# Dao-AILab/flash-attention

Hardware: AMD Instinct MI355X
Metric: attention_fwd_tflops (higher is better)
Workload: dtype bf16; 1 GPU; BASELINE config 3: B=4 H=32 S=4096 D=128 bf16 causal, forward (flash_attn_func path, fa_fwd via C ABI); batch=4, heads=32, seqlen=4096, head_dim=128, causal=True, parallelism=replicas x1

## Files before the change

### flash-attention_amd/csrc/fa_bwd_dkdv_w64.hip

```cpp
#include <cstdlib>
#include <type_traits>

#include "fa_device.h"
#include "fa_kernel_params.h"
#include "fa_launch.h"
#include "fa_fwd_w64_regs.h"
#define FA_W64_CLOB FA_W64_ACC_CLOBBERS_256
#include "fa_w64_asm.h"

#define FA_DKDV64_AHJ 6
#define FA_DKDV64_AHT 3

#ifndef FA_DKDV64_PART
#define FA_DKDV64_PART 0
#endif

namespace fa {
namespace {

template <typename E> FA_DEVINL void kv_mfma_c0(f32x16& d, u32x4 a, u32x4 b) {
  if constexpr (std::is_same<E, __bf16>::value)
    asm volatile("v_mfma_f32_32x32x16_bf16 %0, %1, %2, 0" : "=&v"(d) : "v"(a), "v"(b) : FA_W64_CLOB);
  else
    asm volatile("v_mfma_f32_32x32x16_f16 %0, %1, %2, 0" : "=&v"(d) : "v"(a), "v"(b) : FA_W64_CLOB);
// ... 521 lines not shown
        if constexpr (g == 1) stream_dma_q(c.z);
        if constexpr (g == 3) stream_dma_d(c.z);
        if constexpr (DS && g >= 5 && g <= 11 && (g & 1) == 1) ds_store(ICw<(g - 5) / 2>{});
      });
    } else {
      stream_dma_q(c.z); stream_dma_d(c.z);
      if constexpr (DS) static_for<4>(ds_store);
#pragma unroll
      for (int kb = 0; kb < KB; ++kb)
#pragma unroll
        for (int t = 0; t < 2; ++t) { pc[kb][t] = pn[kb][t]; dc[kb][t] = dn[kb][t]; }
    }
    using Y = ICw<1>; using N = ICw<0>;
    const bool had_prev = c.slot_b != c.slot_a;
    if (__builtin_expect(c.act || had_prev, 1)) {
      if (__builtin_expect(!had_prev, 0)) {
#pragma unroll
        for (int kb = 0; kb < KB; ++kb)
#pragma unroll
          for (int t = 0; t < 2; ++t)
#pragma unroll
            for (int i = 0; i < 4; ++i) {
              unsigned z0, z1;
              asm volatile("v_mov_b32 %0, 0\n\tv_mov_b32 %1, 0" : "=v"(z0), "=v"(z1));
              pc[kb][t][i] = z0; dc[kb][t][i] = z1;
            }
      }
      if (__builtin_expect(c.act && c.msk, 0)) phase_b(Y{}, Y{}, Y{}, c.slot_b, c.q0, pc, dc, pn, dn, c.slot_a);
      else phase_b(Y{}, Y{}, N{}, c.slot_b, c.q0, pc, dc, pn, dn, c.slot_a);
    }
    lds_dma_wait_all();
    stream_store_aux(c.slot2);
    __builtin_amdgcn_sched_barrier(0);
    const int hq_n = (ALIBI || DS) ? (c_left == 1 ? c_h + 1 : c_h) : 0;
    preload_a((st + 1) & 3, hq_n);
    __builtin_amdgcn_sched_barrier(0);
    advance(c, st);
    __builtin_amdgcn_sched_barrier(0);
    __syncthreads();
  };
#pragma unroll 1
  for (int st = 0; st <= n_steps; ++st) step(st);

  char FA_LDS* stage = lds + wave * 32 * (ROW_BYTES + 16);
  mfma_drain_acc();
  static_for<KB>([&](auto kbc) __attribute__((always_inline)) {
    constexpr int kb = decltype(kbc)::value;
    const int kb0 = wk0 + 32 * kb;
    if (kb0 < sk) {
      E* dktile = (E*)p.dk + dk_boff + (k_row0 + kb0) * p.dk_rs + (int64_t)hk * p.dk_hs;
      E* dvtile = (E*)p.dv + dv_boff + (k_row0 + kb0) * p.dv_rs + (int64_t)hk * p.dv_hs;
      f32x16 tt[DB];
      static_for<DB>([&](auto dbc) __attribute__((always_inline)) { acc_read_tuple<16 * (2 * DB + kb * DB + decltype(dbc)::value)>(tt[decltype(dbc)::value]); });
      store_tile_via_lds<E, D>(stage, tt, CAP ? 4.f * p.scale : p.scale, dktile, p.dk_rs, sk - kb0, lane);
      static_for<DB>([&](auto dbc) __attribute__((always_inline)) { acc_read_tuple<16 * (kb * DB + decltype(dbc)::value)>(tt[decltype(dbc)::value]); });
      store_tile_via_lds<E, D>(stage, tt, 1.f, dvtile, p.dv_rs, sk - kb0, lane);
    }
  });
}

#if FA_DKDV64_PART != 2
template <typename E, int D, int FEAT>
__global__ void __launch_bounds__(256, 1) fa_bwd_dkdv_w64_kernel(const BwdK p) {
  dkdv_w64_body<E, D, FEAT, false>(p, blockIdx.x);
}
#endif

#if FA_DKDV64_PART != 1
template <typename E, int D>
static __device__ __forceinline__ void dq_ds_w64_body(const BwdK p, const int cbid) {
  using T = ElemTraits<E>;
  using V8 = typename T::v8;
  constexpr int NW = 4, QB = 2, BM = NW * 64, BN = 64, CPR = D / 8;
  constexpr int ROW_BYTES = D * 2, TILE_K = BN * ROW_BYTES, DB = D / 32;
  constexpr int DS_WAVE = QB * 2 * 2048;
  constexpr int SLOT = TILE_K + NW * DS_WAVE, RING = 3;
  constexpr int RPD = 1024 / ROW_BYTES, DPW = TILE_K / 1024 / NW;
  static_assert(DPW == 4 || DPW == 2, "K pieces per wave");

  extern __shared__ __attribute__((aligned(16))) char smem[];
  char FA_LDS* lds = (char FA_LDS*)smem;
  const int tid = threadIdx.x, lane = tid & 63;
  const int wave = __builtin_amdgcn_readfirstlane(tid >> 6);
  const int hi = lane >> 5;

  const int xcd = cbid & 7, slot_i = cbid >> 3;
  const int per_unit = p.hk_ratio * p.nmb;
  const int jr = slot_i / per_unit, within = slot_i - jr * per_unit;
  const int hg = within / p.nmb, mbr = within - hg * p.nmb;
  const int j = p.c5_cj0 + jr;
  int unit;
  if (p.k_unit_hpx > 0) { const int bb = j / p.k_unit_hpx; unit = bb * (8 * p.k_unit_hpx) + xcd * p.k_unit_hpx + (j - bb * p.k_unit_hpx); }
  else unit = xcd + 8 * j;
  if (unit >= p.k_units) return;
  const int b = unit / p.h_k, hk = unit - b * p.h_k;
  const int h = hk * p.hk_ratio + hg;
  const int m_block = (p.wr >= 0) ? (p.nmb - 1 - mbr) : mbr;
  const int sq = p.sq, sk = p.sk, shift = sk - sq;
  const int m0 = m_block * BM;
  if (m0 >= sq) return;
  const int blk_last = min(m0 + BM, sq) - 1;
  const int kmax = (p.wr >= 0) ? min(sk - 1, blk_last + shift + p.wr) : sk - 1;
  const int n_max = kmax >= 0 ? kmax / BN + 1 : 0;
  const int w_row0 = m0 + wave * 64;

  const E* __restrict__ kp = (const E*)p.k + (int64_t)b * p.k_bs + (int64_t)hk * p.k_hs;
  auto make_srd = [&](const void* base, unsigned long long bytes) __attribute__((always_inline)) {
    const unsigned long long a = (unsigned long long)base;
    u32x4 sd = {(unsigned)__builtin_amdgcn_readfirstlane((unsigned)a), (unsigned)__builtin_amdgcn_readfirstlane((unsigned)(a >> 32)) & 0xffffu,
// ... 89 lines not shown
    if (__builtin_expect(n < n_all, 1)) {
      static_for<4>([&](auto ksc) __attribute__((always_inline)) {
        constexpr int ks = decltype(ksc)::value, kb = ks >> 1, t = ks & 1;
        u32x4 bf[QB];
#pragma unroll
        for (int qb = 0; qb < QB; ++qb) {
          const int a = DOFF + ds_lane + qb * 4096 + kb * 2048 + t * 512;
          bf[qb] = rd_tr(a, a + 256);
        }
        static_for<DB>([&](auto dbc) __attribute__((always_inline)) {
          constexpr int db = decltype(dbc)::value;
          constexpr int kbase = KOFF + kb * 32 * ROW_BYTES + 16 * t * ROW_BYTES;
          const u32x4 af = rd_tr(kbase + (tr_base[0] ^ (db << 6)), kbase + (tr_base[1] ^ (db << 6)));
          kv_mfma_tile<E, db>(af, bf[0]);
          kv_mfma_tile<E, DB + db>(af, bf[1]);
        });
      });
    } else {
      static_for<4>([&](auto ksc) __attribute__((always_inline)) {
        constexpr int ks = decltype(ksc)::value, kb = ks >> 1, t = ks & 1;
        const bool a0 = ds_tile_active(w_row0, n * BN + 32 * kb, sq, sk, shift, p.wl, p.wr), a1 = ds_tile_active(w_row0 + 32, n * BN + 32 * kb, sq, sk, shift, p.wl, p.wr);
        if (a0 || a1) {
          u32x4 bf[QB];
#pragma unroll
          for (int qb = 0; qb < QB; ++qb) {
            const int a = DOFF + ds_lane + qb * 4096 + kb * 2048 + t * 512;
            bf[qb] = rd_tr(a, a + 256);
          }
          static_for<DB>([&](auto dbc) __attribute__((always_inline)) {
            constexpr int db = decltype(dbc)::value;
            constexpr int kbase = KOFF + kb * 32 * ROW_BYTES + 16 * t * ROW_BYTES;
            const u32x4 af = rd_tr(kbase + (tr_base[0] ^ (db << 6)), kbase + (tr_base[1] ^ (db << 6)));
            if (a0) kv_mfma_tile<E, db>(af, bf[0]);
            if (a1) kv_mfma_tile<E, DB + db>(af, bf[1]);
          });
        }
      });
    }
  };
  for (int n = 0; n < n_max; n += RING) {
    tile(ICw<0>{}, n);
    if (n + 1 < n_max) tile(ICw<1>{}, n + 1);
    if (n + 2 < n_max) tile(ICw<2>{}, n + 2);
  }
  __syncthreads();
  mfma_drain_acc();
  E* dqtile = (E*)p.dq + (int64_t)b * p.dq_bs + (int64_t)w_row0 * p.dq_rs + (int64_t)h * p.dq_hs;
  static_for<QB>([&](auto qbc) __attribute__((always_inline)) {
    constexpr int qb = decltype(qbc)::value;
    const int row0 = w_row0 + 32 * qb;
    f32x16 tt[DB];
    static_for<DB>([&](auto dbc) __attribute__((always_inline)) { acc_read_tuple<16 * (qb * DB + decltype(dbc)::value)>(tt[decltype(dbc)::value]); });
    if (row0 < sq)
      store_tile_via_lds<E, D>(lds + (wave * 64 + qb * 32) * (ROW_BYTES + 16), tt, p.scale, dqtile + (int64_t)(32 * qb) * p.dq_rs, p.dq_rs, sq - row0, lane);
  });
}

template <typename E, int D>
__global__ void __launch_bounds__(256, 1) fa_bwd_c5_kernel(const BwdK p) {
  const int bid = blockIdx.x;
  if (bid < p.c5_np) dkdv_w64_body<E, D, 0, true>(p, bid + p.c5_pbid0);
  else dq_ds_w64_body<E, D>(p, bid - p.c5_np);
}

template <typename E, int D>
static int launch_c5_t(const BwdK& p, hipStream_t stream) {
  constexpr int dkdv = 4 * 2 * 32 * D * 2 + 256 * D * 2 + 4 * 2 * 32 * 4 + (D == 128 ? 4 * (D / 16 - 1) * 1024 : 0);
  constexpr int dq = 3 * (64 * D * 2 + 4 * 8192), stage = 256 * (D * 2 + 16);
  constexpr int smem = dkdv > dq ? (dkdv > stage ? dkdv : stage) : (dq > stage ? dq : stage);
  static_assert(smem <= 160 * 1024, "LDS");
  auto kern = fa_bwd_c5_kernel<E, D>;
  static std::atomic<unsigned long long> attr_mask{0};
  if (ensure_dyn_lds(attr_mask, (const void*)kern, 160 * 1024, true) != 0) return -1;
  const long long total = (long long)p.c5_np + p.c5_nc;
  if (total <= 0) return 0;
  hipLaunchKernelGGL(kern, dim3((unsigned)total), dim3(256), smem, stream, p);
  return hipGetLastError() == hipSuccess ? 0 : -1;
}

int launch_bwd_c5(const BwdK& p, int dtype_bf16, int d, hipStream_t stream) {
  if (p.rng != nullptr || p.alibi != nullptr || p.softcap > 0.f || p.d_chunks > 0 || p.cu_q || p.cu_k || p.seqused_q || p.seqused_k || p.k_list) return -2;
  if (p.wl >= 0 || p.sk < p.sq || (d != 128 && d != 64) || (p.c5_np > 0 && !p.ds_ws) || (p.c5_nc > 0 && !p.ds_rd)) return -2;
  const uint64_t span = ((uint64_t)(p.sq > 0 ? p.sq : 1) + 64) * (uint64_t)(p.q_rs > p.do_rs ? p.q_rs : p.do_rs) * 2u;
  const uint64_t kspan = ((uint64_t)p.sk + 128) * (uint64_t)p.k_rs * 2u;
  if (span >= (1ull << 32) || kspan >= (1ull << 32)) return -2;
  if (d == 128) return dtype_bf16 ? launch_c5_t<__bf16, 128>(p, stream) : launch_c5_t<_Float16, 128>(p, stream);
  return dtype_bf16 ? launch_c5_t<__bf16, 64>(p, stream) : launch_c5_t<_Float16, 64>(p, stream);
}
#endif

#if FA_DKDV64_PART != 2
template <typename E, int D, int FEAT>
static int launch_dkdv_w64_f(const BwdK& p, hipStream_t stream) {
  constexpr bool ALIBI = FEAT == FEAT_ALIBI;
  constexpr int base = 4 * 2 * 32 * D * 2 + 256 * D * 2 + 4 * 2 * 32 * 4 + (D == 128 ? 4 * (D / 16 - 1) * 1024 : 0);
  const int smem = base + (ALIBI ? (4 * (p.hk_ratio + 1) + 15) / 16 * 16 : 0);
  if (smem > 160 * 1024) return -2;
  auto kern = fa_bwd_dkdv_w64_kernel<E, D, FEAT>;
  static std::atomic<unsigned long long> attr_mask{0};
  if (ensure_dyn_lds(attr_mask, (const void*)kern, 160 * 1024, true) != 0) return -1;
  const long long total = p.k_list ? (long long)p.k_bound * p.h_k : units_grid(p.k_units, p.k_unit_size);
  if (total <= 0) return 0;
  hipLaunchKernelGGL(kern, dim3((unsigned)total), dim3(256), smem, stream, p);
  return hipGetLastError() == hipSuccess ? 0 : -1;
}
template <typename E, int D>
static int launch_dkdv_w64_t(const BwdK& p, hipStream_t stream) {
// ... 19 lines not shown
```

### flash-attention_amd/csrc/fa_bwd_w64.hip

```cpp
#include <cstdio>
#include <cstdlib>
#include <type_traits>

#include "fa_device.h"
#include "fa_kernel_params.h"
#include "fa_launch.h"
#include "fa_fwd_w64_regs.h"
#define FA_W64_CLOB FA_W64_ACC_CLOBBERS_256
#include "fa_w64_asm.h"

#define FA_BW64_AH 2

namespace fa {
namespace {

constexpr int BW_Q_BASE = 128;
constexpr int BW_DO_BASE = 192;
constexpr float kLog2eW = 1.4426950408889634f;

template <typename E, int BASE> FA_DEVINL void mfma_v_first(f32x16& d, u32x4 a, const f32x16& c) {
  if constexpr (std::is_same<E, __bf16>::value)
    asm volatile("v_mfma_f32_32x32x16_bf16 %0, %1, a[%c3:%c4], %2" : "=&v"(d) : "v"(a), "v"(c), "i"(BASE), "i"(BASE + 3) : FA_W64_CLOB);
  else
    asm volatile("v_mfma_f32_32x32x16_f16 %0, %1, a[%c3:%c4], %2" : "=&v"(d) : "v"(a), "v"(c), "i"(BASE), "i"(BASE + 3) : FA_W64_CLOB);
// ... 560 lines not shown
  auto generic_iter = [&](int u) __attribute__((always_inline)) {
    iter_head(u);
    generic_step(ICw<0>{}, 2 * u - 1, sA, dpA, sB, dpB, fA, fB);
    generic_step(ICw<1>{}, 2 * u, sB, dpB, sA, dpA, fB, fA);
    iter_tail();
  };
  if (n_tiles > 0) {
    int u = 0;
    const int head_end = min(max(uf_lo, 0), n_tiles + 1);
    for (; u < head_end; ++u) generic_iter(u);
    const unsigned wave_dst = (unsigned)(wave * DPW * 1024);
    auto fast_iter = [&](auto maskc, int uu) __attribute__((always_inline)) {
      const int nslot = slot_k == RING - 1 ? 0 : slot_k + 1;
      const unsigned toff_k = (unsigned)(n_min + uu + 1) * (unsigned)(BN * 2) * (unsigned)p.k_rs;
      const unsigned toff_v = (unsigned)(n_min + uu + 1) * (unsigned)(BN * 2) * (unsigned)p.v_rs;
      u32x4 fring[AHK + 1];
      fast_step(ICw<0>{}, maskc, 2 * uu - 1, sA, dpA, sB, dpB, fA, fB, k_srd, koff_l, toff_k,
                __builtin_amdgcn_readfirstlane((unsigned)(nslot * TILE_BYTES) + wave_dst), fring);
      fast_step(ICw<1>{}, maskc, 2 * uu, sB, dpB, sA, dpA, fB, fA, v_srd, voff_l, toff_v,
                __builtin_amdgcn_readfirstlane((unsigned)(V_RING + nslot * TILE_BYTES) + wave_dst), fring);
      have_prev = step_active(2 * uu);
      have_cur = step_active(2 * uu + 1);
      iter_tail();
    };
    int um_lo = uf_lo, um_hi = uf_hi;
    {
      const int f_lo = (w_full_lo - key_base + 31) >> 5;
      const int f_hi = (w_full_hi - 31 - key_base) >> 5;
      um_lo = max(uf_lo, (f_lo + 2) >> 1);
      um_hi = min(uf_hi, f_hi >> 1);
    }
    auto fast_range = [&](auto maskc, int hi_incl) __attribute__((always_inline)) {
      for (; u <= hi_incl; ++u) fast_iter(maskc, u);
    };
    fast_range(ICw<1>{}, min(uf_hi, um_lo - 1));
    fast_range(ICw<0>{}, um_hi);
    fast_range(ICw<1>{}, uf_hi);
    for (; u <= n_tiles; ++u) generic_iter(u);
  }

  if (!wave_valid) return;
  mfma_drain_acc();
  E* dqtile = (E*)p.dq + dq_boff + (q_row0 + w_row0) * p.dq_rs + (int64_t)h * p.dq_hs;
  static_for<QB>([&](auto qbc) __attribute__((always_inline)) {
    constexpr int qb = decltype(qbc)::value;
    f32x16 o_v[DB];
    static_for<DB>([&](auto dbc) __attribute__((always_inline)) {
      constexpr int db = decltype(dbc)::value;
      acc_read_tuple<16 * (qb * DB + db)>(o_v[db]);
    });
    const int row0 = w_row0 + 32 * qb;
    const int lane_e = (int)__builtin_amdgcn_mbcnt_hi(~0u, __builtin_amdgcn_mbcnt_lo(~0u, 0u));
    if (row0 < sq)
      store_tile_via_lds<E, D>(lds + (wave * 64 + qb * 32) * (ROW_BYTES + 16), o_v, CAP ? 4.f * p.scale : p.scale, dqtile + (int64_t)(32 * qb) * p.dq_rs, p.dq_rs,
                               sq - row0, lane_e);
  });
}

template <typename E, int D, bool FUSE_DELTA, int FEAT>
static int launch_bwd_dq_w64_f(const BwdK& p, hipStream_t stream) {
  constexpr int TILE = 64 * D * 2, RINGS = 2 * 3 * TILE, STAGE_IN = 2 * 256 * D * 2, STAGE_OUT = 256 * (D * 2 + 16);
  constexpr int smem = (RINGS > STAGE_IN ? (RINGS > STAGE_OUT ? RINGS : STAGE_OUT) : (STAGE_IN > STAGE_OUT ? STAGE_IN : STAGE_OUT));
  auto kern = fa_bwd_dq_w64_kernel<E, D, FUSE_DELTA, FEAT>;
  static std::atomic<unsigned long long> attr_mask{0};
  if (ensure_dyn_lds(attr_mask, (const void*)kern, smem, true) != 0) return -1;
  const long long total = p.q_list ? (long long)p.q_bound * p.h : units_grid(p.q_units, p.q_unit_size);
  if (total <= 0) return 0;
  hipLaunchKernelGGL(kern, dim3((unsigned)total), dim3(256), smem, stream, p);
  return hipGetLastError() == hipSuccess ? 0 : -1;
}

template <typename E, int D>
static int launch_bwd_dq_w64_t(const BwdK& p, hipStream_t stream) {
  if constexpr (D == 128) {
    if (p.softcap > 0.f) return p.fuse_delta ? launch_bwd_dq_w64_f<E, D, true, FEAT_CAP>(p, stream) : -2;
    if (p.rng) return p.fuse_delta ? launch_bwd_dq_w64_f<E, D, true, FEAT_DROP>(p, stream) : -2;
  } else if (p.softcap > 0.f || p.rng) {
    return -2;
  }
  if (p.alibi) return p.fuse_delta ? launch_bwd_dq_w64_f<E, D, true, FEAT_ALIBI>(p, stream) : launch_bwd_dq_w64_f<E, D, false, FEAT_ALIBI>(p, stream);
  return p.fuse_delta ? launch_bwd_dq_w64_f<E, D, true, 0>(p, stream) : launch_bwd_dq_w64_f<E, D, false, 0>(p, stream);
}

int launch_bwd_dq_w64(const BwdK& p, int dtype_bf16, int d, hipStream_t stream) {
  if ((p.softcap > 0.f) + (p.rng != nullptr) + (p.alibi != nullptr) > 1) return -2;
  if (p.alibi != nullptr && p.wr != 0) return -2;
  const uint64_t span = ((uint64_t)(p.sk > 0 ? p.sk : 1) + 128) * (uint64_t)(p.k_rs > p.v_rs ? p.k_rs : p.v_rs) * 2u;
  if (span >= (1ull << 32)) return -2;
  if (d == 128) return dtype_bf16 ? launch_bwd_dq_w64_t<__bf16, 128>(p, stream) : launch_bwd_dq_w64_t<_Float16, 128>(p, stream);
  if (d == 64) return dtype_bf16 ? launch_bwd_dq_w64_t<__bf16, 64>(p, stream) : launch_bwd_dq_w64_t<_Float16, 64>(p, stream);
  return -2;
}

}
```

### flash-attention_amd/csrc/fa_device.h

```cpp
#pragma once
#include <type_traits>
#include <hip/hip_runtime.h>
#include <stdint.h>

namespace fa {

typedef __attribute__((ext_vector_type(8))) __bf16 bf16x8;
typedef __attribute__((ext_vector_type(8))) _Float16 f16x8;
typedef __attribute__((ext_vector_type(4))) __bf16 bf16x4;
typedef __attribute__((ext_vector_type(4))) _Float16 f16x4;
typedef __attribute__((ext_vector_type(16))) float f32x16;
typedef __attribute__((ext_vector_type(2))) float f32x2;
typedef __attribute__((ext_vector_type(4))) float f32x4;
typedef __attribute__((ext_vector_type(4))) short s16x4;
typedef __attribute__((ext_vector_type(8))) short s16x8;
typedef __attribute__((ext_vector_type(4))) unsigned int u32x4;
typedef __attribute__((ext_vector_type(2))) unsigned int u32x2;

#define FA_DEVINL __device__ __forceinline__
#define FA_LDS __attribute__((address_space(3)))

template <typename E> struct ElemTraits;
template <> struct ElemTraits<__bf16> {
  using v8 = bf16x8;
// ... 26 lines not shown
template <typename E> FA_DEVINL float dot2_acc(unsigned a, unsigned b, float acc) {
  float r;
  if constexpr (std::is_same<E, __bf16>::value) asm("v_dot2_f32_bf16 %0, %1, %2, %3" : "=v"(r) : "v"(a), "v"(b), "v"(acc));
  else asm("v_dot2_f32_f16 %0, %1, %2, %3" : "=v"(r) : "v"(a), "v"(b), "v"(acc));
  return r;
}

FA_DEVINL u32x4 ld_global_16B(const void* p, bool valid) {
  u32x4 z = {0u, 0u, 0u, 0u};
  if (valid) z = *reinterpret_cast<const u32x4*>(p);
  return z;
}

FA_DEVINL void st_global_16B_sc1(void* p, u32x4 x) { asm volatile("global_store_dwordx4 %0, %1, off sc1" ::"v"(p), "v"(x) : "memory"); }

template <typename V> FA_DEVINL V bitcast_u32x4(u32x4 x) { return __builtin_bit_cast(V, x); }

FA_DEVINL s16x4 lds_read_tr16(const char FA_LDS* addr) {
  return __builtin_amdgcn_ds_read_tr16_b64_v4i16((s16x4 FA_LDS*)addr);
}

template <typename V8> FA_DEVINL V8 combine_tr(s16x4 lo, s16x4 hi) {
  s16x8 x = __builtin_shufflevector(lo, hi, 0, 1, 2, 3, 4, 5, 6, 7);
  return __builtin_bit_cast(V8, x);
}

FA_DEVINL void lds_dma_16B(const void* gsrc, const char FA_LDS* lds_dst_uniform) {
  const unsigned dst = __builtin_amdgcn_readfirstlane((unsigned)(unsigned long long)lds_dst_uniform);
  unsigned keep;
  asm volatile("s_mov_b32 %0, m0\n\ts_mov_b32 m0, %2\n\ts_nop 0\n\tglobal_load_lds_dwordx4 %1, off\n\ts_mov_b32 m0, %0"
               : "=&s"(keep)
               : "v"(gsrc), "s"(dst)
               : "memory");
}
FA_DEVINL void lds_dma_wait_all() { asm volatile("s_waitcnt vmcnt(0)" ::: "memory"); }
template <int N> FA_DEVINL void dma_wait() { asm volatile("s_waitcnt vmcnt(%0)" ::"n"(N) : "memory"); }
FA_DEVINL void lds_barrier() { asm volatile("s_waitcnt lgkmcnt(0)\n\ts_barrier" ::: "memory"); }

FA_DEVINL int xcd_interleave(int bid, int n_units, int unit_size, int hpx) {
  constexpr int NX = 8;
  const int xcd = bid % NX, slot = bid / NX;
  const int j = slot / unit_size;
  const int item = slot - j * unit_size;
  int unit;
  if (hpx > 0) {
    const int bb = j / hpx;
    unit = bb * (NX * hpx) + xcd * hpx + (j - bb * hpx);
  } else {
    unit = xcd + NX * j;
  }
  return unit < n_units ? unit * unit_size + item : -1;
}

template <typename E, int D, int DV = D>
FA_DEVINL void store_tile_via_lds(char FA_LDS* stage, const f32x16 (&acc)[DV / 32], float scale, E* gtile, int64_t row_stride,
                                  int rows_valid, int lane, int chunks_valid = DV / 8) {
  using V4 = typename ElemTraits<E>::v4;
  constexpr int ROW_BYTES = D * 2, RS = ROW_BYTES + 16, CPR = D / 8, RPI = 64 / CPR;
  const int qi = lane & 31, hi = lane >> 5;
#pragma unroll
  for (int db = 0; db < DV / 32; ++db)
#pragma unroll
    for (int g = 0; g < 4; ++g) {
      V4 ov;
#pragma unroll
      for (int jj = 0; jj < 4; ++jj) ov[jj] = (E)(acc[db][4 * g + jj] * scale);
      *reinterpret_cast<V4 FA_LDS*>(stage + qi * RS + (32 * db + 8 * g + 4 * hi) * 2) = ov;
    }
#pragma unroll
  for (int i = 0; i < 32 / RPI; ++i) {
    const int row = i * RPI + lane / CPR, ch = lane % CPR;
    const u32x4 x = *reinterpret_cast<const u32x4 FA_LDS*>(stage + row * RS + ch * 16);
    if (row < rows_valid && ch < chunks_valid) *reinterpret_cast<u32x4*>(gtile + (int64_t)row * row_stride + ch * 8) = x;
  }
  asm volatile("s_waitcnt lgkmcnt(0)" ::: "memory");
}

template <typename E, int D, int DV = D>
FA_DEVINL void store_tile_via_lds_packed(char FA_LDS* stage, const f32x16 (&acc)[DV / 32], float scale, E* gbase, int64_t row_stride,
                                         int64_t head_stride, int g, int row0, int rows_total, int lane, int chunks_valid = DV / 8) {
  using V4 = typename ElemTraits<E>::v4;
  constexpr int ROW_BYTES = D * 2, RS = ROW_BYTES + 16, CPR = D / 8, RPI = 64 / CPR;
  const int qi = lane & 31, hi = lane >> 5;
#pragma unroll
  for (int db = 0; db < DV / 32; ++db)
#pragma unroll
    for (int gq = 0; gq < 4; ++gq) {
      V4 ov;
#pragma unroll
      for (int jj = 0; jj < 4; ++jj) ov[jj] = (E)(acc[db][4 * gq + jj] * scale);
      *reinterpret_cast<V4 FA_LDS*>(stage + qi * RS + (32 * db + 8 * gq + 4 * hi) * 2) = ov;
    }
#pragma unroll
  for (int i = 0; i < 32 / RPI; ++i) {
    const int row = i * RPI + lane / CPR, ch = lane % CPR;
    const u32x4 x = *reinterpret_cast<const u32x4 FA_LDS*>(stage + row * RS + ch * 16);
    const int prow = row0 + row, iq = prow / g, hh = prow - iq * g;
    if (prow < rows_total && ch < chunks_valid) *reinterpret_cast<u32x4*>(gbase + (int64_t)iq * row_stride + (int64_t)hh * head_stride + ch * 8) = x;
  }
  asm volatile("s_waitcnt lgkmcnt(0)" ::: "memory");
}

template <int D> FA_DEVINL int swz16(int row) {
  return D >= 128 ? (((row & 3) << 2) | ((row >> 2) & 3)) : ((((row >> 1) & 1) << 2) | ((row >> 2) & 3));
}
template <int D> FA_DEVINL int tile_off(int row, int chunk) { return row * (D * 2) + ((chunk ^ swz16<D>(row)) << 4); }

FA_DEVINL bool ds_tile_active(int q0, int k0, int sq, int sk, int shift, int wl, int wr) {
  if (q0 >= sq || k0 >= sk) return false;
  const int k1 = min(k0 + 31, sk - 1);
  if (wr >= 0 && k0 > q0 + 31 + shift + wr) return false;
  if (wl >= 0 && k1 < q0 + shift - wl) return false;
  return true;
}
FA_DEVINL int ds_slot(int key, int hi) { return (key & 3) | (hi << 2) | ((key >> 2) << 3); }
__host__ __device__ inline int ds_row_start(int i, int a, int jb, int np64) {
  const int m = i < jb ? i : jb;
  const int n1 = a + m - 1, n0 = a - 1;
  return 2 * (((n1 * n1) >> 2) - ((n0 * n0) >> 2) + (i > jb ? i - jb : 0) * np64);
}

// ... 63 lines not shown
```

### flash-attention_amd/csrc/fa_fwd_w64.hip

```cpp
#include <cstdio>
#include <cstdlib>
#include <type_traits>

#include "fa_device.h"
#include "fa_kernel_params.h"
#include "fa_launch.h"
#include "fa_fwd_w64_regs.h"
#define FA_W64_CLOB FA_W64_ACC_CLOBBERS
#include "fa_w64_asm.h"


#define FA_W64_AH 3
#define FA_W64_KDMA_G0 0
#define FA_W64_KDMA_GS 2
#define FA_W64_VDMA_G0 1
#define FA_W64_VDMA_GS 2

namespace fa {

template <int D> FA_DEVINL constexpr int k_swz_w(int row) { return D == 128 ? (row & 15) : ((row >> 1) & 7); }
template <int D> FA_DEVINL constexpr int v_swz_w(int row) { return D == 128 ? (row & 3) : ((row >> 1) & 1); }

#define FA_W64_MFMA(E_) (std::is_same<E_, __bf16>::value ? "v_mfma_f32_32x32x16_bf16" : "v_mfma_f32_32x32x16_f16")
constexpr int W64_Q_BASE = 128;
// ... 233 lines not shown
  auto dma_tile = [&](auto isvc, int buf, int t) __attribute__((always_inline)) {
    constexpr bool ISV = decltype(isvc)::value != 0;
    const bool real = t >= 0 && t < n_tiles;
    const int64_t rs = ISV ? p.v_rs : p.k_rs;
    const unsigned lds_dst = (unsigned)((ISV ? 2 + buf : buf) * TILE_BYTES + wave * DPW * 1024);
    if constexpr (PAGED) {
      const int n = n_min + t, page = max(n, 0) / pg_tpp;
      const u32x4 sd = real ? tile_srd(isvc, page_entry(page), max(n, 0) - page * pg_tpp, n) : null_srd;
      dma_pieces(sd, ISV ? voff_l : koff_l, lds_dst);
      return;
    }
    const unsigned toff = real ? (unsigned)(n_min + t) * (unsigned)(BN * 2) * (unsigned)rs : 0u;
    unsigned vo[DPW];
#pragma unroll
    for (int i = 0; i < DPW; ++i) vo[i] = (ISV ? voff_l[i] : koff_l[i]) + toff;
    dma_pieces(real ? (ISV ? v_srd : k_srd) : null_srd, vo, lds_dst);
  };

  __syncthreads();
  if (q_in_lds != vb) dma_q(q_srd_of(blk));
  if (n_tiles > 0) dma_tile(ICw<0>{}, 0, tile_of(0));
  if (q_in_lds != vb) {
    if (n_tiles > 0) { if constexpr (DPW == 4) asm volatile("s_waitcnt vmcnt(4)" ::: "memory"); else asm volatile("s_waitcnt vmcnt(2)" ::: "memory"); }
    else lds_dma_wait_all();
  }
  {
    const float cq = SOFTCAP ? p.scale * 2.885390081777927f / p.softcap : p.scale_log2;
    u32x4 qraw[QB][KS];
#pragma unroll
    for (int qb = 0; qb < QB; ++qb)
#pragma unroll
      for (int ks = 0; ks < KS; ++ks) {
        const int qbase = Q_OFF + (wave * 64 + qb * 32 + qi) * ROW_BYTES + ((hi ^ k_swz_w<D>(qi)) << 4);
        qraw[qb][ks] = *(const u32x4 FA_LDS*)(unsigned long)(unsigned)(qbase ^ (ks << 5));
      }
    auto load_q = [&](auto qbc, auto ksc) __attribute__((always_inline)) {
      constexpr int qb = decltype(qbc)::value, ks = decltype(ksc)::value;
      const V8 raw = bitcast_u32x4<V8>(qraw[qb][ks]);
      V8 sc;
#pragma unroll
      for (int j = 0; j < 8; j += 2) {
        typedef __attribute__((ext_vector_type(2))) float f32x2;
        f32x2 pr = {(float)raw[j], (float)raw[j + 1]};
        pr *= f32x2{cq, cq};
        sc[j] = (E)pr[0]; sc[j + 1] = (E)pr[1];
      }
      acc_write_frag<W64_Q_BASE + 4 * (qb * KS + ks)>(__builtin_bit_cast(u32x4, sc));
    };
    auto load_q_all = [&](auto qbc) __attribute__((always_inline)) {
      load_q(qbc, ICw<0>{}); load_q(qbc, ICw<1>{}); load_q(qbc, ICw<2>{}); load_q(qbc, ICw<3>{});
      if constexpr (KS == 8) { load_q(qbc, ICw<4>{}); load_q(qbc, ICw<5>{}); load_q(qbc, ICw<6>{}); load_q(qbc, ICw<7>{}); }
    };
    load_q_all(ICw<0>{});
    if (n_tiles > 0) dma_tile(ICw<1>{}, 1, -1);
    load_q_all(ICw<1>{});
  }
  lds_dma_wait_all();
  __syncthreads();
  u32x4 qn_srd = null_srd;
  int qn_done = QDMA, qn_per_iter = QDMA;
  {
    q_in_lds = -1;
    if (nxt_id_ok && fill_blk(nxt)) {
      asm volatile("s_waitcnt lgkmcnt(0)" ::: "memory");
      qn_srd = q_srd_of(nxt); qn_done = 0;
      qn_per_iter = n_tiles >= QDMA ? 1 : n_tiles >= QDMA / 2 ? 2 : n_tiles >= QDMA / 4 ? 4 : QDMA;
      if (n_tiles == 0) { dma_q(qn_srd); lds_dma_wait_all(); qn_done = QDMA; }
      q_in_lds = vb + (int)gridDim.x;
    }
  }
  auto q_trickle = [&]() __attribute__((always_inline)) {
    if (qn_done < QDMA) {
#pragma unroll 1
      for (int j = 0; j < qn_per_iter; ++j) dma_q_piece(qn_srd, qn_done + j);
      qn_done += qn_per_iter;
    }
  };

  const int kbase = qi * ROW_BYTES + ((hi ^ k_swz_w<D>(qi)) << 4);
  const int tr_i = lane & 15, tr_half = (lane >> 4) & 1;
  const int tr_rr = tr_i >> 2, tr_cc = tr_i & 3;
  const int vbase = (4 * hi + tr_rr) * ROW_BYTES + (v_swz_w<D>(tr_rr) << 6) + tr_half * 32 + tr_cc * 8;
  int ka[KS], va[DB];
#pragma unroll
  for (int ks = 0; ks < KS; ++ks) ka[ks] = kbase ^ (ks << 5);
#pragma unroll
  for (int db = 0; db < DB; ++db) va[db] = vbase ^ (db << 6);

  {
    u32x4 zf = {0u, 0u, 0u, 0u};
    asm volatile("" : "+v"(zf));
    acc_zero_tuples_mfma<0>(zf, std::make_integer_sequence<int, 2 * DB>{});
  }
  float m_run[QB], l_run[QB][2], o_lag[QB];
  float thr_l[QB];
  float capc = 0.f, cap_m2c = 0.f, capoff[QB] = {0.f, 0.f};
  if constexpr (SOFTCAP) {
    capc = __builtin_bit_cast(float, __builtin_amdgcn_readfirstlane(__builtin_bit_cast(int, p.softcap * 1.4426950408889634f)));
    cap_m2c = -2.f * capc;
    capoff[0] = capc; capoff[1] = capc;
  }
  unsigned drop_kr[7] = {0u, 0u, 0u, 0u, 0u, 0u, 0u}, drop_thr = 255u, drop_row[QB] = {0u, 0u};
  if constexpr (DROP) {
    const unsigned k0_ = (unsigned)__builtin_amdgcn_readfirstlane((int)drop_bh_key(p.rng, b * p.h + h));
#pragma unroll
    for (int r = 0; r < 7; ++r) drop_kr[r] = k0_ + (unsigned)r * 0x9E3779B9u;
    drop_thr = (unsigned)__builtin_amdgcn_readfirstlane((int)p.drop_thr8);
// ... 363 lines not shown
    if constexpr (PM != 2) { if (__builtin_expect(masked(), 0)) clear_mask(2 * u + 2); }
    iter_end();
  };
  auto idle_iter = [&](int u) __attribute__((always_inline)) {
    q_trickle();
    dma_tile(ICw<0>{}, (u & 1) ^ 1, tile_of(u + 1)); dma_tile(ICw<1>{}, u & 1, tile_of(u));
    iter_end();
  };
  if (n_tiles > 0) {
    const bool active = u_first <= u_last;
    const int ua = active ? (u_first & ~1) : n_tiles + 1;
    int u = 0;
#pragma unroll 1
    for (; u < ua; ++u) idle_iter(u);
    if (active) {
      pg_enter(u);
      if constexpr (ALIBI) { if (u > 0) clear_mask(2 * u); }
      if constexpr (FEAT == 0) {
        step_pair(ICw<0>{}, u, ICw<1>{}); ++u;
#pragma unroll 1
        for (;;) {
          if (u >= u_last) break;
          step_pair(ICw<1>{}, u, ICw<0>{}); ++u;
          if (u >= u_last) break;
          step_pair(ICw<0>{}, u, ICw<0>{}); ++u;
        }
        if (u & 1) step_pair(ICw<1>{}, u, ICw<2>{}); else step_pair(ICw<0>{}, u, ICw<2>{});
        ++u;
      } else {
#pragma unroll 1
        for (;;) {
          step_pair(ICw<0>{}, u, ICw<0>{}); ++u;
          if (u > u_last) break;
          step_pair(ICw<1>{}, u, ICw<0>{}); ++u;
          if (u > u_last) break;
        }
      }
    }
#pragma unroll 1
    for (; u <= n_tiles; ++u) idle_iter(u);
  }

  if (wave_valid) {
  mfma_drain_acc();
  u32x4 o_srd;
  {
    const int rows = min(BM, sq - m0);
    const unsigned long long a = (unsigned long long)(op + (int64_t)m0 * p.o_rs);
    const unsigned lo = __builtin_amdgcn_readfirstlane((unsigned)a);
    const unsigned hi16 = __builtin_amdgcn_readfirstlane((unsigned)(a >> 32)) & 0xffffu;
    const unsigned nr = __builtin_amdgcn_readfirstlane((unsigned)(((unsigned long long)(rows - 1) * (unsigned long long)p.o_rs + D) * 2ull));
    o_srd = u32x4{lo, hi16, nr, 0x00020000u};
  }
  static_for<QB>([&](auto qbc) __attribute__((always_inline)) {
    constexpr int qb = decltype(qbc)::value;
    f32x16 o_v[DB];
    static_for<DB>([&](auto dbc) __attribute__((always_inline)) {
      constexpr int db = decltype(dbc)::value;
      acc_read_tuple<16 * (qb * DB + db)>(o_v[db]);
#pragma unroll
      for (int r = 0; r < 16; ++r) o_v[db][r] = o_v[db][r];
    });
    const float l_tot = half_sum(l_run[qb][0] + l_run[qb][1]);
    const bool dead = (l_tot == 0.f) || (l_tot != l_tot);
    const float inv = (dead ? 1.f : 1.f / l_tot) * o_lag[qb] * (DROP ? p.rp_keep : 1.f);
    const int row0 = w_row0 + 32 * qb;
    if (row0 < sq) {
      {
        using V4 = typename T::v4;
        constexpr int RS = ROW_BYTES + 16, RPI = 64 / CPR;
        char FA_LDS* stage = lds + (wave * 64 + qb * 32) * RS;
#pragma unroll
        for (int db = 0; db < DB; ++db)
#pragma unroll
          for (int g = 0; g < 4; ++g) {
            V4 ov;
#pragma unroll
            for (int jj = 0; jj < 4; ++jj) ov[jj] = (E)(o_v[db][4 * g + jj] * inv);
            *reinterpret_cast<V4 FA_LDS*>(stage + qi * RS + (32 * db + 8 * g + 4 * hi) * 2) = ov;
          }
        unsigned lane_off = (unsigned)(((wave * 64 + lane / CPR) * (int)p.o_rs + (lane % CPR) * 8) * 2);
        asm volatile("" : "+v"(lane_off));
#pragma unroll
        for (int i = 0; i < 32 / RPI; ++i) {
          const u32x4 x = *reinterpret_cast<const u32x4 FA_LDS*>(stage + (i * RPI + lane / CPR) * RS + (lane % CPR) * 16);
          const unsigned soff = __builtin_amdgcn_readfirstlane((unsigned)((qb * 32 + i * RPI) * (int)p.o_rs * 2));
          asm volatile("buffer_store_dwordx4 %0, %1, %2, %3 offen" : : "v"(x), "v"(lane_off), "s"(o_srd), "s"(soff) : "memory");
        }
        asm volatile("s_waitcnt lgkmcnt(0)" ::: "memory");
      }
      const int my_row = row0 + qi;
      if (my_row < sq && hi == 0) lsep[my_row] = dead ? INFINITY : (m_run[qb] * kLn2 + __logf(l_tot));
    }
  });
  }
  }
}

template <typename E, int D, int FEAT = 0, bool PAGED = false>
static int launch_fwd_w64_t(const FwdK& p, hipStream_t stream) {
  constexpr int STAGE = 256 * (D * 2 + 16);
  constexpr int smem = ((4 * 64 * D * 2 > STAGE ? 4 * 64 * D * 2 : STAGE + 1023) / 1024 * 1024) + 256 * D * 2;
  auto kern = fa_fwd_w64_kernel<E, D, FEAT, PAGED>;
  static std::atomic<unsigned long long> attr_mask{0};
  if (ensure_dyn_lds(attr_mask, (const void*)kern, smem, true) != 0) return -1;
  const long long total = p.work_list ? (long long)p.work_bound * p.h : units_grid(p.n_units, p.unit_size);
  if (total <= 0) return 0;
  FwdK pp = p;
  long long grid = total;
  const int cus = device_cu_count();
  const bool balanced = p.wr < 0 || (p.unit_size > 1 && (cus / 8) % p.unit_size == 0);
  if (!p.work_list && cus >= 8 && total > cus && balanced && knobs().w64_persist != 0) {
    grid = cus / 8 * 8;
    pp.persist_total = (int)total;
  }
  hipLaunchKernelGGL(kern, dim3((unsigned)grid), dim3(256), smem, stream, pp);
  if (hipGetLastError() != hipSuccess) return -1;
  LastSchedule& ls = last_schedule();
  ls.fwd_kernel = 3; ls.fwd_nw = 4; ls.fwd_feat = FEAT; ls.fwd_splits = 1; ls.fwd_list = p.work_list != nullptr; ls.d = D;
  ls.bf16 = std::is_same<E, __bf16>::value;
  if (FEAT) snprintf(ls.name, sizeof(ls.name), "fa::fa_fwd_w64_kernel<%s,%d,%s>", ls.bf16 ? "bf16" : "f16", D, FEAT == FEAT_CAP ? "softcap" : FEAT == FEAT_DROP ? "dropout" : "alibi");
  else if (PAGED) snprintf(ls.name, sizeof(ls.name), "fa::fa_fwd_w64_kernel<%s,%d,paged>", ls.bf16 ? "bf16" : "f16", D);
  else snprintf(ls.name, sizeof(ls.name), "fa::fa_fwd_w64_kernel<%s,%d>", ls.bf16 ? "bf16" : "f16", D);
  return 0;
}

#ifndef FA_W64_PART
#define FA_W64_PART 0
#endif
int launch_fwd_w64_bf16(const FwdK& p, int d, hipStream_t stream);
int launch_fwd_w64_f16(const FwdK& p, int d, hipStream_t stream);
#if FA_W64_PART != 1
int launch_fwd_w64_f16(const FwdK& p, int d, hipStream_t stream) {
  if (p.rng) {
    if (d == 128) return launch_fwd_w64_t<_Float16, 128, FEAT_DROP>(p, stream);
    if (d == 64) return launch_fwd_w64_t<_Float16, 64, FEAT_DROP>(p, stream);
    return -2;
  }
  if (p.softcap > 0.f) {
    if (d == 128) return launch_fwd_w64_t<_Float16, 128, FEAT_CAP>(p, stream);
    if (d == 64) return launch_fwd_w64_t<_Float16, 64, FEAT_CAP>(p, stream);
    return -2;
  }
  if (p.alibi) {
    if (d == 128) return launch_fwd_w64_t<_Float16, 128, FEAT_ALIBI>(p, stream);
    if (d == 64) return launch_fwd_w64_t<_Float16, 64, FEAT_ALIBI>(p, stream);
    return -2;
// ... 53 lines not shown
```

Baseline: 1095 TFLOP/s.

## Batch LDS reads before global stores in epilogues and overlap forward output conversion

Adds a BATCH mode to store_tile_via_lds that issues all LDS reads, waits once, then issues all global stores, and enables it in the backward dq/dk/dv epilogues. The forward epilogue is restructured so both Q blocks' outputs are scaled and converted up front with packed multiplies, and the LDS staging of block 1 is interleaved with the buffer stores of block 0. It also drops the early prefetch of K/V tile 1 in the non-feature forward prologue. The aim is to cut per-store LDS wait serialization in the epilogue, at the cost of more live registers and a changed prologue prefetch pattern.

```diff
diff --git a/flash-attention_amd/csrc/fa_bwd_dkdv_w64.hip b/flash-attention_amd/csrc/fa_bwd_dkdv_w64.hip
--- a/flash-attention_amd/csrc/fa_bwd_dkdv_w64.hip
+++ b/flash-attention_amd/csrc/fa_bwd_dkdv_w64.hip
@@ -597,9 +597,9 @@
       E* dvtile = (E*)p.dv + dv_boff + (k_row0 + kb0) * p.dv_rs + (int64_t)hk * p.dv_hs;
       f32x16 tt[DB];
       static_for<DB>([&](auto dbc) __attribute__((always_inline)) { acc_read_tuple<16 * (2 * DB + kb * DB + decltype(dbc)::value)>(tt[decltype(dbc)::value]); });
-      store_tile_via_lds<E, D>(stage, tt, CAP ? 4.f * p.scale : p.scale, dktile, p.dk_rs, sk - kb0, lane);
+      store_tile_via_lds<E, D, D, true>(stage, tt, CAP ? 4.f * p.scale : p.scale, dktile, p.dk_rs, sk - kb0, lane);
       static_for<DB>([&](auto dbc) __attribute__((always_inline)) { acc_read_tuple<16 * (kb * DB + decltype(dbc)::value)>(tt[decltype(dbc)::value]); });
-      store_tile_via_lds<E, D>(stage, tt, 1.f, dvtile, p.dv_rs, sk - kb0, lane);
+      store_tile_via_lds<E, D, D, true>(stage, tt, 1.f, dvtile, p.dv_rs, sk - kb0, lane);
     }
   });
 }
@@ -795,7 +795,7 @@
     f32x16 tt[DB];
     static_for<DB>([&](auto dbc) __attribute__((always_inline)) { acc_read_tuple<16 * (qb * DB + decltype(dbc)::value)>(tt[decltype(dbc)::value]); });
     if (row0 < sq)
-      store_tile_via_lds<E, D>(lds + (wave * 64 + qb * 32) * (ROW_BYTES + 16), tt, p.scale, dqtile + (int64_t)(32 * qb) * p.dq_rs, p.dq_rs, sq - row0, lane);
+      store_tile_via_lds<E, D, D, true>(lds + (wave * 64 + qb * 32) * (ROW_BYTES + 16), tt, p.scale, dqtile + (int64_t)(32 * qb) * p.dq_rs, p.dq_rs, sq - row0, lane);
   });
 }
 
diff --git a/flash-attention_amd/csrc/fa_bwd_w64.hip b/flash-attention_amd/csrc/fa_bwd_w64.hip
--- a/flash-attention_amd/csrc/fa_bwd_w64.hip
+++ b/flash-attention_amd/csrc/fa_bwd_w64.hip
@@ -636,7 +636,7 @@
     const int row0 = w_row0 + 32 * qb;
     const int lane_e = (int)__builtin_amdgcn_mbcnt_hi(~0u, __builtin_amdgcn_mbcnt_lo(~0u, 0u));
     if (row0 < sq)
-      store_tile_via_lds<E, D>(lds + (wave * 64 + qb * 32) * (ROW_BYTES + 16), o_v, CAP ? 4.f * p.scale : p.scale, dqtile + (int64_t)(32 * qb) * p.dq_rs, p.dq_rs,
+      store_tile_via_lds<E, D, D, true>(lds + (wave * 64 + qb * 32) * (ROW_BYTES + 16), o_v, CAP ? 4.f * p.scale : p.scale, dqtile + (int64_t)(32 * qb) * p.dq_rs, p.dq_rs,
                                sq - row0, lane_e);
   });
 }
diff --git a/flash-attention_amd/csrc/fa_device.h b/flash-attention_amd/csrc/fa_device.h
--- a/flash-attention_amd/csrc/fa_device.h
+++ b/flash-attention_amd/csrc/fa_device.h
@@ -102,7 +102,7 @@
   return unit < n_units ? unit * unit_size + item : -1;
 }
 
-template <typename E, int D, int DV = D>
+template <typename E, int D, int DV = D, bool BATCH = false>
 FA_DEVINL void store_tile_via_lds(char FA_LDS* stage, const f32x16 (&acc)[DV / 32], float scale, E* gtile, int64_t row_stride,
                                   int rows_valid, int lane, int chunks_valid = DV / 8) {
   using V4 = typename ElemTraits<E>::v4;
@@ -117,6 +117,19 @@
       for (int jj = 0; jj < 4; ++jj) ov[jj] = (E)(acc[db][4 * g + jj] * scale);
       *reinterpret_cast<V4 FA_LDS*>(stage + qi * RS + (32 * db + 8 * g + 4 * hi) * 2) = ov;
     }
+  if constexpr (BATCH) {
+    u32x4 x[32 / RPI];
+#pragma unroll
+    for (int i = 0; i < 32 / RPI; ++i) x[i] = *reinterpret_cast<const u32x4 FA_LDS*>(stage + (i * RPI + lane / CPR) * RS + (lane % CPR) * 16);
+    __builtin_amdgcn_s_waitcnt(0xC07F);
+    __builtin_amdgcn_sched_barrier(0);
+#pragma unroll
+    for (int i = 0; i < 32 / RPI; ++i) {
+      const int row = i * RPI + lane / CPR, ch = lane % CPR;
+      if (row < rows_valid && ch < chunks_valid) *reinterpret_cast<u32x4*>(gtile + (int64_t)row * row_stride + ch * 8) = x[i];
+    }
+    return;
+  }
 #pragma unroll
   for (int i = 0; i < 32 / RPI; ++i) {
     const int row = i * RPI + lane / CPR, ch = lane % CPR;
diff --git a/flash-attention_amd/csrc/fa_fwd_w64.hip b/flash-attention_amd/csrc/fa_fwd_w64.hip
--- a/flash-attention_amd/csrc/fa_fwd_w64.hip
+++ b/flash-attention_amd/csrc/fa_fwd_w64.hip
@@ -309,7 +309,7 @@
       if constexpr (KS == 8) { load_q(qbc, ICw<4>{}); load_q(qbc, ICw<5>{}); load_q(qbc, ICw<6>{}); load_q(qbc, ICw<7>{}); }
     };
     load_q_all(ICw<0>{});
-    if (n_tiles > 0) dma_tile(ICw<1>{}, 1, -1);
+    if constexpr (FEAT != 0) { if (n_tiles > 0) dma_tile(ICw<1>{}, 1, -1); }
     load_q_all(ICw<1>{});
   }
   lds_dma_wait_all();
@@ -779,47 +779,73 @@
     const unsigned nr = __builtin_amdgcn_readfirstlane((unsigned)(((unsigned long long)(rows - 1) * (unsigned long long)p.o_rs + D) * 2ull));
     o_srd = u32x4{lo, hi16, nr, 0x00020000u};
   }
-  static_for<QB>([&](auto qbc) __attribute__((always_inline)) {
-    constexpr int qb = decltype(qbc)::value;
-    f32x16 o_v[DB];
-    static_for<DB>([&](auto dbc) __attribute__((always_inline)) {
-      constexpr int db = decltype(dbc)::value;
-      acc_read_tuple<16 * (qb * DB + db)>(o_v[db]);
-#pragma unroll
-      for (int r = 0; r < 16; ++r) o_v[db][r] = o_v[db][r];
-    });
-    const float l_tot = half_sum(l_run[qb][0] + l_run[qb][1]);
-    const bool dead = (l_tot == 0.f) || (l_tot != l_tot);
-    const float inv = (dead ? 1.f : 1.f / l_tot) * o_lag[qb] * (DROP ? p.rp_keep : 1.f);
-    const int row0 = w_row0 + 32 * qb;
-    if (row0 < sq) {
-      {
-        using V4 = typename T::v4;
-        constexpr int RS = ROW_BYTES + 16, RPI = 64 / CPR;
-        char FA_LDS* stage = lds + (wave * 64 + qb * 32) * RS;
-#pragma unroll
-        for (int db = 0; db < DB; ++db)
-#pragma unroll
-          for (int g = 0; g < 4; ++g) {
-            V4 ov;
-#pragma unroll
-            for (int jj = 0; jj < 4; ++jj) ov[jj] = (E)(o_v[db][4 * g + jj] * inv);
-            *reinterpret_cast<V4 FA_LDS*>(stage + qi * RS + (32 * db + 8 * g + 4 * hi) * 2) = ov;
+  {
+    using V4 = typename T::v4;
+    typedef __attribute__((ext_vector_type(2))) float f32x2;
+    constexpr int RS = ROW_BYTES + 16, RPI = 64 / CPR, NST = 32 / RPI;
+    float l_tot[QB];
+    bool dead[QB];
+    V4 ov[QB][DB][4];
+    auto convert = [&](auto qbc) __attribute__((always_inline)) {
+      constexpr int qb = decltype(qbc)::value;
+      f32x16 o_v[DB];
+      static_for<DB>([&](auto dbc) __attribute__((always_inline)) {
+        constexpr int db = decltype(dbc)::value;
+        acc_read_tuple<16 * (qb * DB + db)>(o_v[db]);
+      });
+      l_tot[qb] = half_sum(l_run[qb][0] + l_run[qb][1]);
+      dead[qb] = (l_tot[qb] == 0.f) || (l_tot[qb] != l_tot[qb]);
+      const float inv = (dead[qb] ? 1.f : 1.f / l_tot[qb]) * o_lag[qb] * (DROP ? p.rp_keep : 1.f);
+#pragma unroll
+      for (int db = 0; db < DB; ++db)
+#pragma unroll
+        for (int g = 0; g < 4; ++g)
+#pragma unroll
+          for (int jj = 0; jj < 4; jj += 2) {
+            f32x2 pr = {o_v[db][4 * g + jj], o_v[db][4 * g + jj + 1]};
+            pr *= f32x2{inv, inv};
+            ov[qb][db][g][jj] = (E)pr[0]; ov[qb][db][g][jj + 1] = (E)pr[1];
           }
-        unsigned lane_off = (unsigned)(((wave * 64 + lane / CPR) * (int)p.o_rs + (lane % CPR) * 8) * 2);
-        asm volatile("" : "+v"(lane_off));
-#pragma unroll
-        for (int i = 0; i < 32 / RPI; ++i) {
-          const u32x4 x = *reinterpret_cast<const u32x4 FA_LDS*>(stage + (i * RPI + lane / CPR) * RS + (lane % CPR) * 16);
-          const unsigned soff = __builtin_amdgcn_readfirstlane((unsigned)((qb * 32 + i * RPI) * (int)p.o_rs * 2));
-          asm volatile("buffer_store_dwordx4 %0, %1, %2, %3 offen" : : "v"(x), "v"(lane_off), "s"(o_srd), "s"(soff) : "memory");
-        }
-        asm volatile("s_waitcnt lgkmcnt(0)" ::: "memory");
-      }
-      const int my_row = row0 + qi;
-      if (my_row < sq && hi == 0) lsep[my_row] = dead ? INFINITY : (m_run[qb] * kLn2 + __logf(l_tot));
-    }
-  });
+    };
+    auto stage = [&](auto qbc, u32x4 (&x)[NST]) __attribute__((always_inline)) {
+      constexpr int qb = decltype(qbc)::value;
+      char FA_LDS* stage_p = lds + (wave * 64 + qb * 32) * RS;
+#pragma unroll
+      for (int db = 0; db < DB; ++db)
+#pragma unroll
+        for (int g = 0; g < 4; ++g) *reinterpret_cast<V4 FA_LDS*>(stage_p + qi * RS + (32 * db + 8 * g + 4 * hi) * 2) = ov[qb][db][g];
+#pragma unroll
+      for (int i = 0; i < NST; ++i) x[i] = *reinterpret_cast<const u32x4 FA_LDS*>(stage_p + (i * RPI + lane / CPR) * RS + (lane % CPR) * 16);
+      __builtin_amdgcn_sched_barrier(0);
+    };
+    unsigned lane_off = (unsigned)(((wave * 64 + lane / CPR) * (int)p.o_rs + (lane % CPR) * 8) * 2);
+    asm volatile("" : "+v"(lane_off));
+    auto store = [&](auto qbc, const u32x4 (&x)[NST], const u32x4& srd, unsigned voff) __attribute__((always_inline)) {
+      constexpr int qb = decltype(qbc)::value;
+#pragma unroll
+      for (int i = 0; i < NST; ++i) {
+        const unsigned soff = __builtin_amdgcn_readfirstlane((unsigned)((qb * 32 + i * RPI) * (int)p.o_rs * 2));
+        asm volatile("buffer_store_dwordx4 %0, %1, %2, %3 offen" : : "v"(x[i]), "v"(voff), "s"(srd), "s"(soff) : "memory");
+      }
+    };
+    auto put_lse = [&](auto qbc) __attribute__((always_inline)) {
+      constexpr int qb = decltype(qbc)::value;
+      const int my_row = w_row0 + 32 * qb + qi;
+      if (my_row < sq && hi == 0) lsep[my_row] = dead[qb] ? INFINITY : (m_run[qb] * kLn2 + __logf(l_tot[qb]));
+    };
+    u32x4 x0[NST], x1[NST];
+    convert(ICw<0>{});
+    stage(ICw<0>{}, x0);
+    convert(ICw<1>{});
+    __builtin_amdgcn_sched_barrier(0);
+    store(ICw<0>{}, x0, o_srd, lane_off);
+    put_lse(ICw<0>{});
+    if (w_row0 + 32 < sq) {
+      stage(ICw<1>{}, x1);
+      store(ICw<1>{}, x1, o_srd, lane_off);
+      put_lse(ICw<1>{});
+    }
+  }
   }
   }
 }
```

Result: no change. 1095 TFLOP/s (median of 2 runs) (-0.0%).
